# neoyinyao/Recommender

Measured on AMD Instinct MI355X. Metric: examples/sec fwd+bwd, Criteo-DLRM 26×40M×128 batch 65536, 1/2/4/8 GPU, higher is better.
Workload: dtype fp32; 1 GPU; dlrm_criteo_26x40000000x128; global_batch=65536, per_gpu_batch=65536, rows=40000000, dim=128, slots=26, optimizer=sgd, parallelism=single, prefetch=False

## Files before the change

recommender_amd/csrc/embedding.hip:

```cpp
#include <cstdlib>

#include "common.hpp"

namespace rs {

int32_t radix_sort_pairs(uint32_t*, int32_t*, uint32_t*, int32_t*, int64_t, int64_t, void*, size_t,
                         hipStream_t);
size_t radix_sort_ws_size(int64_t);
int32_t exclusive_scan_i32(const int32_t*, int32_t*, int64_t, int32_t*, void*, size_t, hipStream_t);
size_t exclusive_scan_ws_size(int64_t);

template <int VEC>
struct RowIO;
template <>
struct RowIO<4> {
  static __device__ __forceinline__ void load(const float* p, float (&v)[4]) {
    float4 t = *reinterpret_cast<const float4*>(p);
    v[0] = t.x; v[1] = t.y; v[2] = t.z; v[3] = t.w;
  }
  static __device__ __forceinline__ void store(float* p, const float (&v)[4]) {
    *reinterpret_cast<float4*>(p) = make_float4(v[0], v[1], v[2], v[3]);
  }
};
template <int VEC>
// ... 257 lines not shown

__device__ __forceinline__ int32_t seg_id_of(const ApplyArgs& a, const uint32_t* keys, int64_t k) {
  bool head = (k == 0) || keys[k - 1] != keys[k];
  return a.seg_excl ? a.seg_excl[k] + (head ? 1 : 0) - 1 : 0;
}

#ifndef RS_APPLY_BLOCKS_PER_CU
#define RS_APPLY_BLOCKS_PER_CU (1 << 20)
#endif
constexpr int kApplyBlocksPerCU = RS_APPLY_BLOCKS_PER_CU;

template <int OPT, int VEC, int CPL>
__device__ __forceinline__ void seg_tile_one(const uint32_t* __restrict__ keys,
                                             const int32_t* __restrict__ pos, int64_t n,
                                             uint32_t n_rows, const float* __restrict__ grad,
                                             const ApplyArgs& a, int lpr_log2, int64_t t);

template <int OPT, int VEC, int CPL>
__global__ __launch_bounds__(256) void seg_tile_kernel(const uint32_t* __restrict__ keys,
                                                       const int32_t* __restrict__ pos, int64_t n,
                                                       uint32_t n_rows, const float* __restrict__ grad,
                                                       ApplyArgs a, int lpr_log2, int64_t n_tiles) {
  const int gpb = blockDim.x >> lpr_log2;
  const int64_t groups = (int64_t)gridDim.x * gpb;
  for (int64_t t = (int64_t)blockIdx.x * gpb + (threadIdx.x >> lpr_log2); t < n_tiles; t += groups)
    seg_tile_one<OPT, VEC, CPL>(keys, pos, n, n_rows, grad, a, lpr_log2, t);
}

template <int OPT, int VEC, int CPL>
__device__ __forceinline__ void seg_tile_one(const uint32_t* __restrict__ keys,
                                             const int32_t* __restrict__ pos, int64_t n,
                                             uint32_t n_rows, const float* __restrict__ grad,
                                             const ApplyArgs& a, int lpr_log2, int64_t t) {
  constexpr int T = RS_DEDUP_TILE;
  constexpr int U = 8;
  const int lpr = 1 << lpr_log2;
  const int gl = threadIdx.x & (lpr - 1);
  const int64_t k0 = t * T;
  const int64_t k1 = k0 + T < n ? k0 + T : n;
  const int dim = a.dim;

  uint32_t run_row = keys[k0];
  int64_t run_start = k0;
  bool run_starts = (k0 == 0) || keys[k0 - 1] != run_row;
  const float* grad0 = (OPT == OPT_DENSE && a.n_gseg > 0) ? a.gseg[0] : grad;
  float acc[CPL][VEC];
#pragma unroll
  for (int c = 0; c < CPL; ++c)
#pragma unroll
    for (int e = 0; e < VEC; ++e) acc[c][e] = 0.f;

  auto emit = [&](uint32_t row, bool starts, bool ends, int64_t head_k) {
    if (row >= n_rows) return;
    if (starts && ends) {
      finalize_row<OPT, VEC, CPL>(a, row, gl, lpr, acc, OPT == OPT_EMIT ? seg_id_of(a, keys, head_k) : 0);
    } else {
      float* dst = a.partial + ((t * 2) + (starts ? 1 : 0)) * (int64_t)dim;
#pragma unroll
      for (int c = 0; c < CPL; ++c) {
        int col = (gl + c * lpr) * VEC;
        if (col < dim) RowIO<VEC>::store(dst + col, acc[c]);
      }
    }
  };

  for (int64_t kb = k0; kb < k1; kb += U) {
    float r[U][CPL][VEC];
    float sc[U];
    uint32_t kk[U];
    uint32_t kr[U];
    int32_t pr[U];
#pragma unroll
    for (int u = 0; u < U; ++u) {
      const int64_t k = kb + u < k1 ? kb + u : k0;
      kr[u] = keys[k];
      pr[u] = pos[k];
    }
    const float* rsp = a.row_scale ? a.row_scale : grad0;
    float sr[U];
#pragma unroll
    for (int u = 0; u < U; ++u) {
      const bool valid = kb + u < k1;
      kk[u] = valid ? kr[u] : 0xFFFFFFFFu;
      const int64_t p = valid ? pr[u] : 0;
      const bool live = valid && kk[u] < n_rows;
      sr[u] = rsp[a.row_scale && live ? p / a.scale_group : 0];
#pragma unroll
      for (int c = 0; c < CPL; ++c) {
        int col = (gl + c * lpr) * VEC;
        const bool ok = live && col < dim;
        if constexpr (OPT == OPT_DENSE)
          load_stream<VEC>(ok ? dense_grad_row(a, grad, p, dim) + col : grad0, r[u][c]);
        else
          load_stream<VEC>(ok ? grad + p * dim + col : grad0, r[u][c]);
      }
    }
#pragma unroll
    for (int u = 0; u < U; ++u) sc[u] = a.row_scale ? sr[u] : 1.f;
#pragma unroll
    for (int u = 0; u < U; ++u) {
      int64_t k = kb + u;
      if (k < k1) {
        if (kk[u] != run_row) {
          emit(run_row, run_starts, true, run_start);
#pragma unroll
          for (int c = 0; c < CPL; ++c)
#pragma unroll
            for (int e = 0; e < VEC; ++e) acc[c][e] = 0.f;
          run_row = kk[u];
          run_starts = true;
          run_start = k;
        }
        if (a.row_scale) {
#pragma unroll
          for (int c = 0; c < CPL; ++c)
#pragma unroll
            for (int e = 0; e < VEC; ++e) acc[c][e] += __fmul_rn(sc[u], r[u][c][e]);
        } else {
#pragma unroll
          for (int c = 0; c < CPL; ++c)
#pragma unroll
            for (int e = 0; e < VEC; ++e) acc[c][e] += r[u][c][e];
        }
      }
    }
  }
  bool ends = (k1 >= n) || keys[k1] != run_row;
  emit(run_row, run_starts, ends, run_start);
  if (gl == 0) {
    uint8_t f = 0;
    if (!ends && run_starts && run_row < n_rows) f |= 1;
    const uint32_t fk = keys[k0];
    if ((t % 32) == 0 && k0 > 0 && fk < n_rows && keys[k0 - 1] == fk) f |= 2;
    a.tile_flags[t] = f;
  }
}

struct Tile32Edges {
  uint32_t last_row;
  bool last_open;
  bool first_cont;
  uint32_t first_key;
};

template <int OPT, int Q = 0>
__device__ __forceinline__ Tile32Edges tile32_walk(const uint32_t* __restrict__ keys,
                                                   const int32_t* __restrict__ pos, int64_t n,
                                                   uint32_t n_rows, const float* __restrict__ grad,
                                                   const ApplyArgs& a, int64_t t, float* pbase) {
  constexpr int T = 32, VEC = 4, CPL = 1, U = 8;
  constexpr bool kQueue = Q > 0 && OPT == OPT_SGD;
  constexpr int QN = Q > 0 ? Q : 1;
  const int gl = threadIdx.x & 31;
  const int64_t k0 = t * T;
  const int64_t k1 = k0 + T < n ? k0 + T : n;
  const int ne = (int)(k1 - k0);
  const int dim = a.dim;
  const int col = gl * VEC;
  const bool mine = gl < ne;
  const uint32_t klo = a.key_lo, kspan = n_rows - a.key_lo;
  auto key_ok = [&](uint32_t k) { return k - klo < kspan; };
  const int64_t ki = k0 + (mine ? gl : 0);
  const uint32_t kraw = keys[ki];
  const int32_t praw = pos[ki];
  const uint32_t kbraw = keys[k0 > 0 ? k0 - 1 : 0];
  const uint32_t karaw = keys[k1 < n ? k1 : n - 1];
  const uint32_t kv = mine ? kraw : 0xFFFFFFFFu;
  const int32_t pv = mine ? praw : 0;
  const bool lv = mine && key_ok(kv);
  const uint32_t key_before = k0 > 0 ? kbraw : 0xFFFFFFFFu;
  const uint32_t key_after = k1 < n ? karaw : 0xFFFFFFFEu;
  float sv = 1.f;
  if (a.row_scale) sv = a.row_scale[(lv ? pv : 0) / a.scale_group];
  auto key_of = [&](int u) { return (uint32_t)__shfl((int)kv, u, 32); };
  auto load_batch = [&](int b0, float (&r)[U][VEC]) {
#pragma unroll
    for (int u = 0; u < U; ++u) {
      const int e = b0 + u;
      const int32_t p = __shfl(pv, e, 32);
      const bool live = e < ne && key_ok(key_of(e));
      load_stream<VEC>(grad + (live ? (int64_t)p * dim : 0) + col, r[u]);
    }
  };
  uint32_t run_row = key_of(0);
  int run_start = 0;
  bool run_starts = run_row != key_before;
  float acc[CPL][VEC];
#pragma unroll
  for (int c = 0; c < VEC; ++c) acc[0][c] = 0.f;
  uint32_t qrow[QN];
  float qacc[QN][VEC];
  int qn = 0;
  auto flush = [&]() {
    if constexpr (kQueue) {
      float tr[QN][VEC];
#pragma unroll
      for (int i = 0; i < QN; ++i) {
        const uint32_t rr = i < qn ? qrow[i] : (qn > 0 ? qrow[0] : 0u);
        RowIO<VEC>::load(a.table + (int64_t)rr * dim + col, tr[i]);
      }
#pragma unroll
      for (int i = 0; i < QN; ++i) {
        if (i < qn) {
#pragma unroll
          for (int c = 0; c < VEC; ++c) tr[i][c] = tr[i][c] - a.p.lr * qacc[i][c];
          RowIO<VEC>::store(a.table + (int64_t)qrow[i] * dim + col, tr[i]);
        }
      }
      qn = 0;
    }
  };
  auto emit = [&](uint32_t row, bool starts, bool ends, int head_e) {
    if (!key_ok(row)) return;
    if (starts && ends) {
      if constexpr (kQueue) {
        if (qn == QN) flush();
#pragma unroll
        for (int i = 0; i < QN; ++i) {
          if (i == qn) {
            qrow[i] = row;
#pragma unroll
            for (int c = 0; c < VEC; ++c) qacc[i][c] = acc[0][c];
          }
        }
        ++qn;
      } else {
        finalize_row<OPT, VEC, CPL>(a, row, gl, 32, acc, OPT == OPT_EMIT ? seg_id_of(a, keys, k0 + head_e) : 0);
      }
    } else {
      RowIO<VEC>::store(pbase + (starts ? 1 : 0) * dim + col, acc[0]);
    }
  };
  float rA[U][VEC], rB[U][VEC];
  load_batch(0, rA);
  auto consume = [&](int b0, float (&r)[U][VEC]) {
#pragma unroll
    for (int u = 0; u < U; ++u) {
      const int e = b0 + u;
      if (e < ne) {
        const uint32_t ku = key_of(e);
        if (ku != run_row) {
          emit(run_row, run_starts, true, run_start);
#pragma unroll
          for (int c = 0; c < VEC; ++c) acc[0][c] = 0.f;
          run_row = ku;
          run_starts = true;
          run_start = e;
        }
        if (a.row_scale) {
          const float sc = __shfl(sv, e, 32);
#pragma unroll
          for (int c = 0; c < VEC; ++c) acc[0][c] += __fmul_rn(sc, r[u][c]);
        } else {
#pragma unroll
          for (int c = 0; c < VEC; ++c) acc[0][c] += r[u][c];
        }
      }
    }
  };
#ifndef RS_T32_SINGLE
  load_batch(U, rB);
  consume(0, rA);
  if (ne > 2 * U) load_batch(2 * U, rA);
  consume(U, rB);
  if (ne > 3 * U) load_batch(3 * U, rB);
  if (ne > 2 * U) consume(2 * U, rA);
  if (ne > 3 * U) consume(3 * U, rB);
#else
  consume(0, rA);
  for (int b0 = U; b0 < ne; b0 += U) {
    load_batch(b0, rA);
    consume(b0, rA);
  }
#endif
  const bool ends = key_after != run_row;
  emit(run_row, run_starts, ends, run_start);
  flush();
  Tile32Edges ed;
  ed.last_row = run_row;
  ed.last_open = !ends && run_starts && key_ok(run_row);
  ed.first_key = key_of(0);
  ed.first_cont = k0 > 0 && key_ok(ed.first_key) && key_before == ed.first_key;
  return ed;
}

template <int OPT>
__global__ __launch_bounds__(256) void seg_tile32_kernel(const uint32_t* __restrict__ keys,
                                                         const int32_t* __restrict__ pos, int64_t n,
                                                         uint32_t n_rows,
                                                         const float* __restrict__ grad,
                                                         ApplyArgs a, int64_t n_tiles) {
  const int64_t t = (int64_t)blockIdx.x * 8 + (threadIdx.x >> 5);
  if (t >= n_tiles) return;
  const Tile32Edges e = tile32_walk<OPT>(keys, pos, n, n_rows, grad, a, t,
                                         a.partial + t * 2 * (int64_t)a.dim);
  if ((threadIdx.x & 31) == 0) {
    uint8_t f = 0;
    if (e.last_open) f |= 1;
    if ((t % 32) == 0 && e.first_cont) f |= 2;
    a.tile_flags[t] = f;
  }
}

template <int OPT, int Q = 0>
__global__ __launch_bounds__(1024) void seg_group32_kernel(const uint32_t* __restrict__ keys,
                                                           const int32_t* __restrict__ pos,
                                                           int64_t n, uint32_t n_rows,
                                                           const float* __restrict__ grad,
                                                           ApplyArgs a, int64_t n_tiles) {
  constexpr int G = 32, D = 128, T = 32;
  __shared__ __attribute__((aligned(16))) float ps[G][2][D];
  __shared__ uint32_t fkey[G];
  __shared__ int skip;
  const int gi = threadIdx.x >> 5, gl = threadIdx.x & 31;
  const int64_t t = (int64_t)blockIdx.x * G + gi;
  const bool live = t < n_tiles;
  if (a.ranged) {
    if (threadIdx.x == 0) {
      const int64_t f = (int64_t)blockIdx.x * G * T;
      const int64_t l = (f + (int64_t)G * T < n ? f + (int64_t)G * T : n) - 1;
      skip = f < n && (keys[l] < a.key_lo || keys[f] >= n_rows);
    }
    __syncthreads();
    if (skip) {
      if (gl == 0 && live) a.tile_flags[t] = 0;
      return;
    }
  }
  Tile32Edges e{};
  if (live) e = tile32_walk<OPT, Q>(keys, pos, n, n_rows, grad, a, t, &ps[gi][0][0]);
  if (gl == 0) fkey[gi] = live ? e.first_key : 0xFFFFFFFFu;
  __syncthreads();
  if (!live) return;
  const int col = gl * 4;
  uint8_t gflag = 0;
  if (e.last_open) {
    const uint32_t row = e.last_row;
    float acc[1][4];
    {
      const float4 h = *reinterpret_cast<const float4*>(&ps[gi][1][col]);
      acc[0][0] = h.x; acc[0][1] = h.y; acc[0][2] = h.z; acc[0][3] = h.w;
    }
    int u = gi + 1;
    for (; u < G && fkey[u] == row; ++u) {
      const float4 c = *reinterpret_cast<const float4*>(&ps[u][0][col]);
      acc[0][0] += c.x; acc[0][1] += c.y; acc[0][2] += c.z; acc[0][3] += c.w;
    }
    const int64_t tn = ((int64_t)blockIdx.x + 1) * G;
    const bool crosses = u == G && tn < n_tiles && keys[tn * T] == row;
    if (crosses) {
      RowIO<4>::store(a.chunk + (t * 2 + 1) * (int64_t)D + col, acc[0]);
      gflag = 1;
    } else {
      finalize_row<OPT, 4, 1>(a, row, gl, 32, acc,
                              OPT == OPT_EMIT ? seg_id_of(a, keys, t * T + T - 1) : 0);
    }
  }
  if (gi == 0 && e.first_cont) {
    const uint32_t fk = e.first_key;
    float acc[4];
    {
      const float4 h = *reinterpret_cast<const float4*>(&ps[0][0][col]);
      acc[0] = h.x; acc[1] = h.y; acc[2] = h.z; acc[3] = h.w;
    }
    for (int u = 1; u < G && fkey[u] == fk; ++u) {
      const float4 c = *reinterpret_cast<const float4*>(&ps[u][0][col]);
      acc[0] += c.x; acc[1] += c.y; acc[2] += c.z; acc[3] += c.w;
    }
    RowIO<4>::store(a.chunk + (t * 2) * (int64_t)D + col, acc);
  }
  if (gl == 0) a.tile_flags[t] = gflag;
}

constexpr int kFixChunk = 32;

template <int VEC, int CPL>
__device__ __forceinline__ void load_or_zero(const float* p, int dim, int gl, int lpr,
                                             float (&acc)[CPL][VEC]) {
#pragma unroll
  for (int c = 0; c < CPL; ++c) {
    int col = (gl + c * lpr) * VEC;
    if (col < dim) {
      RowIO<VEC>::load(p + col, acc[c]);
    } else {
#pragma unroll
      for (int e = 0; e < VEC; ++e) acc[c][e] = 0.f;
    }
  }
}

template <int VEC, int CPL>
__device__ __forceinline__ void store_row(float* p, int dim, int gl, int lpr,
                                          const float (&acc)[CPL][VEC]) {
#pragma unroll
  for (int c = 0; c < CPL; ++c) {
    int col = (gl + c * lpr) * VEC;
    if (col < dim) RowIO<VEC>::store(p + col, acc[c]);
  }
}

template <int VEC, int CPL>
__device__ __forceinline__ void fold_group(const uint32_t* keys, int64_t n, uint32_t key,
                                           const float* part, int64_t t1, int64_t t_end, int dim,
                                           int gl, int lpr, float (&acc)[CPL][VEC]) {
  constexpr int T = RS_DEDUP_TILE;
  constexpr int U = 8;
  for (int64_t t = t1; t < t_end; t += U) {
    bool in[U];
    float r[U][CPL][VEC];
#pragma unroll
    for (int u = 0; u < U; ++u) {
      const int64_t tt = t + u;
      in[u] = tt < t_end && tt * T < n && keys[tt * T] == key;
    }
    bool more = true;
#pragma unroll
    for (int u = 0; u < U; ++u) {
      more = more && in[u];
      in[u] = more;
    }
#pragma unroll
    for (int u = 0; u < U; ++u) {
      if (in[u]) {
        load_or_zero<VEC, CPL>(part + ((t + u) * 2) * (int64_t)dim, dim, gl, lpr, r[u]);
      }
    }
#pragma unroll
    for (int u = 0; u < U; ++u)
      if (in[u])
#pragma unroll
        for (int c = 0; c < CPL; ++c)
#pragma unroll
          for (int e = 0; e < VEC; ++e) acc[c][e] += r[u][c][e];
    if (!more) return;
  }
}

template <int VEC, int CPL>
__global__ __launch_bounds__(256) void seg_chunk_kernel(const uint32_t* __restrict__ keys, int64_t n,
                                                        uint32_t n_rows, ApplyArgs a, int lpr_log2,
                                                        int64_t n_tiles, float* __restrict__ chunk) {
  constexpr int T = RS_DEDUP_TILE;
  const int lpr = 1 << lpr_log2;
  const int gl = threadIdx.x & (lpr - 1);
  const int64_t t = (int64_t)blockIdx.x * (blockDim.x >> lpr_log2) + (threadIdx.x >> lpr_log2);
  if (t >= n_tiles) return;
  const uint8_t flags = a.tile_flags[t];
  if (flags == 0) return;
  const int dim = a.dim;
  const int64_t k0 = t * T;
  const int64_t klast = (k0 + T < n ? k0 + T : n) - 1;
  const int64_t group_end = (t / kFixChunk + 1) * kFixChunk;
  float acc[CPL][VEC];
  if (flags & 1) {
    const uint32_t lk = keys[klast];
    load_or_zero<VEC, CPL>(a.partial + (t * 2 + 1) * (int64_t)dim, dim, gl, lpr, acc);
    fold_group<VEC, CPL>(keys, n, lk, a.partial, t + 1, group_end, dim, gl, lpr, acc);
    store_row<VEC, CPL>(chunk + (t * 2 + 1) * (int64_t)dim, dim, gl, lpr, acc);
  }
  if (flags & 2) {
    const uint32_t fk = keys[k0];
    load_or_zero<VEC, CPL>(a.partial + (t * 2) * (int64_t)dim, dim, gl, lpr, acc);
    fold_group<VEC, CPL>(keys, n, fk, a.partial, t + 1, group_end, dim, gl, lpr, acc);
    store_row<VEC, CPL>(chunk + (t * 2) * (int64_t)dim, dim, gl, lpr, acc);
  }
}

template <int OPT, int VEC, int CPL>
__device__ __forceinline__ void fixup_one(const uint32_t* __restrict__ keys, const ApplyArgs& a,
                                          int lpr_log2, int64_t n_tiles,
                                          const float* __restrict__ chunk, int64_t t);

template <int OPT, int VEC, int CPL>
__global__ __launch_bounds__(256) void seg_fixup_kernel(const uint32_t* __restrict__ keys, int64_t n,
                                                        uint32_t n_rows, ApplyArgs a, int lpr_log2,
                                                        int64_t n_tiles,
                                                        const float* __restrict__ chunk) {
  const int64_t t = (int64_t)blockIdx.x * (blockDim.x >> lpr_log2) + (threadIdx.x >> lpr_log2);
  if (t >= n_tiles - 1) return;
  if (!(a.tile_flags[t] & 1)) return;
  fixup_one<OPT, VEC, CPL>(keys, a, lpr_log2, n_tiles, chunk, t);
}

template <int OPT, int VEC, int CPL>
__global__ __launch_bounds__(256) void seg_fixup_wave_kernel(const uint32_t* __restrict__ keys,
                                                             ApplyArgs a, int lpr_log2,
                                                             int64_t n_tiles,
                                                             const float* __restrict__ chunk) {
  constexpr int T = RS_DEDUP_TILE;
  constexpr int U = 16;
  const int64_t t = (int64_t)blockIdx.x * 4 + (threadIdx.x >> 6);
  if (t >= n_tiles - 1) return;
  if (!(a.tile_flags[t] & 1)) return;
  const int lane = threadIdx.x & 63;
  const int lpr = 1 << lpr_log2;
  const int nlg = 64 >> lpr_log2;
  const int lg = lane >> lpr_log2, gl = lane & (lpr - 1);
  const int64_t klast = t * T + T - 1;
  const uint32_t row = keys[klast];
  const int dim = a.dim;
  float acc[CPL][VEC];
  load_or_zero<VEC, CPL>(chunk + (t * 2 + 1) * (int64_t)dim, dim, gl, lpr, acc);
  const int span = nlg * U < 64 ? nlg * U : 64;
  for (int64_t g = t / kFixChunk + 1;; g += span) {
    uint32_t k[U];
    float r[U][CPL][VEC];
    uint32_t mine = 0;
#pragma unroll
    for (int u = 0; u < U; ++u) {
      const int64_t gg = g + (int64_t)lg * U + u;
      const int64_t tt = gg * kFixChunk;
      const bool in = lg * U + u < span && tt < n_tiles;
      k[u] = in ? keys[tt * T] : ~row;
      if (in)
        load_or_zero<VEC, CPL>(chunk + (tt * 2) * (int64_t)dim, dim, gl, lpr, r[u]);
      else
#pragma unroll
        for (int c = 0; c < CPL; ++c)
#pragma unroll
          for (int e = 0; e < VEC; ++e) r[u][c][e] = 0.f;
      mine |= (k[u] == row ? 1u : 0u) << u;
    }
    uint64_t w = 0;
    for (int src = 0; src < nlg && src * U < span; ++src)
      w |= (uint64_t)(uint32_t)__shfl((int)mine, src * lpr) << (src * U);
    const int nrun = ~w == 0ull ? 64 : (int)__builtin_ctzll(~w);
    for (int src = 0; src < nlg && src * U < nrun; ++src) {
#pragma unroll
      for (int u = 0; u < U; ++u) {
        float v[CPL][VEC];
#pragma unroll
        for (int c = 0; c < CPL; ++c)
#pragma unroll
          for (int e = 0; e < VEC; ++e) v[c][e] = __shfl(r[u][c][e], src * lpr + gl);
        if (src * U + u < nrun)
#pragma unroll
          for (int c = 0; c < CPL; ++c)
#pragma unroll
            for (int e = 0; e < VEC; ++e) acc[c][e] += v[c][e];
      }
    }
    if (nrun < span) break;
  }
  if (lg == 0) finalize_row<OPT, VEC, CPL>(a, row, gl, lpr, acc, OPT == OPT_EMIT ? seg_id_of(a, keys, klast) : 0);
}

template <int OPT>
__global__ __launch_bounds__(256) void seg_fixup_sweep_kernel(const uint32_t* __restrict__ keys,
                                                              ApplyArgs a, int64_t n_tiles,
                                                              const float* __restrict__ chunk) {
  const int gl = threadIdx.x & 31;
  const int64_t groups = (int64_t)gridDim.x * 8;
  for (int64_t t0 = ((int64_t)blockIdx.x * 8 + (threadIdx.x >> 5)) * 32; t0 < n_tiles - 1;
       t0 += groups * 32) {
    const int64_t tl = t0 + gl;
    const bool head = tl < n_tiles - 1 && (a.tile_flags[tl] & 1);
    uint32_t bits = (uint32_t)(__ballot(head) >> (threadIdx.x & 32));
    while (bits) {
      const int u = __builtin_ctz(bits);
      bits &= bits - 1;
      fixup_one<OPT, 4, 1>(keys, a, 5, n_tiles, chunk, t0 + u);
    }
  }
}

template <int OPT, int VEC, int CPL>
__device__ __forceinline__ void fixup_one(const uint32_t* __restrict__ keys, const ApplyArgs& a,
                                          int lpr_log2, int64_t n_tiles,
                                          const float* __restrict__ chunk, int64_t t) {
  constexpr int T = RS_DEDUP_TILE;
  constexpr int U = 16;
  const int lpr = 1 << lpr_log2;
  const int gl = threadIdx.x & (lpr - 1);
  const int64_t klast = t * T + T - 1;
  const uint32_t row = keys[klast];
  const int dim = a.dim;
  float acc[CPL][VEC];
  load_or_zero<VEC, CPL>(chunk + (t * 2 + 1) * (int64_t)dim, dim, gl, lpr, acc);
  for (int64_t g = t / kFixChunk + 1;; g += U) {
    bool in[U];
    float r[U][CPL][VEC];
    bool more = true;
    uint32_t k[U];
#pragma unroll
    for (int u = 0; u < U; ++u) {
      const int64_t tt = (g + u) * kFixChunk;
      k[u] = tt < n_tiles ? keys[tt * T] : ~row;
      if (tt < n_tiles)
        load_or_zero<VEC, CPL>(chunk + ((g + u) * kFixChunk * 2) * (int64_t)dim, dim, gl, lpr, r[u]);
    }
#pragma unroll
    for (int u = 0; u < U; ++u) {
      in[u] = more && k[u] == row;
      more = in[u];
    }
#pragma unroll
    for (int u = 0; u < U; ++u)
      if (in[u])
#pragma unroll
        for (int c = 0; c < CPL; ++c)
#pragma unroll
          for (int e = 0; e < VEC; ++e) acc[c][e] += r[u][c][e];
    if (!more) break;
  }
  finalize_row<OPT, VEC, CPL>(a, row, gl, lpr, acc, OPT == OPT_EMIT ? seg_id_of(a, keys, klast) : 0);
}

__global__ void head_flags_kernel(const uint32_t* __restrict__ keys, int64_t n, uint32_t n_rows,
                                  int32_t* __restrict__ flags) {
  int64_t i = blockIdx.x * (int64_t)blockDim.x + threadIdx.x;
  int64_t stride = (int64_t)gridDim.x * blockDim.x;
  for (; i < n; i += stride) {
    uint32_t k = keys[i];
    flags[i] = (k < n_rows && (i == 0 || keys[i - 1] != k)) ? 1 : 0;
  }
}

__device__ __forceinline__ void keras_decay(float& w, float& m, float& v, float lr, float b1,
                                            float b2, float eps) {
  const float m1 = m * b1;
  const float v1 = v * b2;
  const float upd = (lr * m1) / (sqrtf(v1) + eps);
  m = m1;
  v = v1;
  w = w - upd;
}

template <int VEC>
__device__ __forceinline__ bool keras_state_zero(const float (&mm)[VEC], const float (&vv)[VEC]) {
  bool z = true;
#pragma unroll
  for (int e = 0; e < VEC; ++e) z &= (__float_as_uint(mm[e]) == 0u) & (vv[e] == 0.0f);
  return z;
}

template <int VEC>
__global__ __launch_bounds__(256) void keras_dense_sweep_kernel(float* __restrict__ w,
                                                                float* __restrict__ m,
                                                                float* __restrict__ v, int64_t n_rows,
                                                                int dim, rs_adam_params p,
                                                                const uint32_t* __restrict__ bitmap) {
  const int64_t chunks_per_row = dim / VEC;
  const int64_t total = n_rows * chunks_per_row;
  int64_t i = blockIdx.x * (int64_t)blockDim.x + threadIdx.x;
  const int64_t stride = (int64_t)gridDim.x * blockDim.x;
  for (; i < total; i += stride) {
    int64_t row = i / chunks_per_row;
    if ((bitmap[row >> 5] >> (row & 31)) & 1u) continue;
    int64_t off = i * VEC;
    float ww[VEC], mm[VEC], vv[VEC];
    RowIO<VEC>::load(m + off, mm);
    RowIO<VEC>::load(v + off, vv);
    if (keras_state_zero<VEC>(mm, vv)) continue;
    RowIO<VEC>::load(w + off, ww);
#pragma unroll
    for (int e = 0; e < VEC; ++e) keras_decay(ww[e], mm[e], vv[e], p.lr, p.beta1, p.beta2, p.epsilon);
    RowIO<VEC>::store(w + off, ww);
    RowIO<VEC>::store(m + off, mm);
    RowIO<VEC>::store(v + off, vv);
  }
}

template <int VEC>
__device__ __forceinline__ void keras_replay_row(float* w, float* m, float* v, int64_t r, int dim,
                                                 int gl, int lpr, int32_t from, int32_t to,
                                                 const float* lr_hist, float b1, float b2,
                                                 float eps) {
  for (int col = gl * VEC; col < dim; col += lpr * VEC) {
    const int64_t off = r * dim + col;
    float ww[VEC], mm[VEC], vv[VEC];
    RowIO<VEC>::load(m + off, mm);
    RowIO<VEC>::load(v + off, vv);
    if (keras_state_zero<VEC>(mm, vv)) continue;
    RowIO<VEC>::load(w + off, ww);
    for (int32_t st = from; st <= to; ++st) {
      const float lr = lr_hist[st];
#pragma unroll
      for (int e = 0; e < VEC; ++e) keras_decay(ww[e], mm[e], vv[e], lr, b1, b2, eps);
    }
    RowIO<VEC>::store(w + off, ww);
    RowIO<VEC>::store(m + off, mm);
    RowIO<VEC>::store(v + off, vv);
  }
}

template <int VEC>
__global__ __launch_bounds__(256) void keras_catchup_kernel(
    float* __restrict__ w, float* __restrict__ m, float* __restrict__ v, int32_t* __restrict__ last,
    uint32_t n_rows, int dim, const uint32_t* __restrict__ rows, int64_t n,
    const float* __restrict__ lr_hist, int32_t step, float b1, float b2, float eps, int lpr_log2) {
  const int lpr = 1 << lpr_log2;
  const int gl = threadIdx.x & (lpr - 1);
  const int64_t stride = ((int64_t)gridDim.x * blockDim.x) >> lpr_log2;
  for (int64_t i = ((int64_t)blockIdx.x * blockDim.x + threadIdx.x) >> lpr_log2; i < n; i += stride) {
    const uint32_t r = rows[i];
    if (r >= n_rows || (i > 0 && rows[i - 1] == r)) continue;
    const int32_t l0 = last[r];
    if (l0 + 1 <= step - 1)
      keras_replay_row<VEC>(w, m, v, r, dim, gl, lpr, l0 + 1, step - 1, lr_hist, b1, b2, eps);
    if (gl == 0) last[r] = step - 1;
  }
}

__global__ __launch_bounds__(256) void keras_mark_kernel(int32_t* __restrict__ last, uint32_t n_rows,
                                                          const uint32_t* __restrict__ rows,
                                                          int64_t n, int32_t step) {
  for (int64_t i = (int64_t)blockIdx.x * blockDim.x + threadIdx.x; i < n;
       i += (int64_t)gridDim.x * blockDim.x) {
    const uint32_t r = rows[i];
    if (r < n_rows && (i == 0 || rows[i - 1] != r)) last[r] = step;
  }
}

template <int VEC>
__global__ __launch_bounds__(256) void keras_materialize_kernel(
    float* __restrict__ w, float* __restrict__ m, float* __restrict__ v, int32_t* __restrict__ last,
    int64_t n_rows, int dim, const float* __restrict__ lr_hist, int32_t step, float b1, float b2,
    float eps, int lpr_log2) {
  const int lpr = 1 << lpr_log2;
  const int gl = threadIdx.x & (lpr - 1);
  const int64_t stride = ((int64_t)gridDim.x * blockDim.x) >> lpr_log2;
  for (int64_t r = ((int64_t)blockIdx.x * blockDim.x + threadIdx.x) >> lpr_log2; r < n_rows; r += stride) {
    const int32_t l0 = last[r];
    if (l0 + 1 <= step)
      keras_replay_row<VEC>(w, m, v, r, dim, gl, lpr, l0 + 1, step, lr_hist, b1, b2, eps);
    if (gl == 0) last[r] = step;
  }
}

template <template <int, int> class K>
struct Noop {};

#define RS_DISPATCH_VEC_CPL(geom, CALL)                                   \
  do {                                                                    \
    switch ((geom).vec * 100 + (geom).cpl) {                              \
      case 401: { constexpr int VEC = 4, CPL = 1; CALL; } break;          \
      case 402: { constexpr int VEC = 4, CPL = 2; CALL; } break;          \
      case 404: { constexpr int VEC = 4, CPL = 4; CALL; } break;          \
      case 408: { constexpr int VEC = 4, CPL = 8; CALL; } break;          \
      case 201: { constexpr int VEC = 2, CPL = 1; CALL; } break;          \
      case 202: { constexpr int VEC = 2, CPL = 2; CALL; } break;          \
      case 204: { constexpr int VEC = 2, CPL = 4; CALL; } break;          \
      case 101: { constexpr int VEC = 1, CPL = 1; CALL; } break;          \
      case 102: { constexpr int VEC = 1, CPL = 2; CALL; } break;          \
      case 104: { constexpr int VEC = 1, CPL = 4; CALL; } break;          \
      default:                                                            \
        set_error("row geometry vec=%d cpl=%d unsupported (dim too large)", (geom).vec, (geom).cpl); \
        return RS_E_UNSUPPORTED;                                          \
    }                                                                     \
  } while (0)

__global__ __launch_bounds__(256) void keras_bitmap_mark_kernel(const uint32_t* __restrict__ keys,
                                                               int64_t n, uint32_t n_rows,
                                                               uint32_t* __restrict__ bitmap) {
  for (int64_t k = (int64_t)blockIdx.x * 256 + threadIdx.x; k < n; k += (int64_t)gridDim.x * 256) {
    const uint32_t row = keys[k];
    if (row < n_rows && (k == 0 || keys[k - 1] != row)) atomicOr(bitmap + (row >> 5), 1u << (row & 31));
  }
}

#ifndef RS_SGD_QUEUE
#define RS_SGD_QUEUE 2
#endif

static int32_t launch_segments(int opt, const uint32_t* keys, const int32_t* pos, int64_t n,
                               int64_t n_rows, const float* grad, const ApplyArgs& a,
                               const RowGeom& geom, hipStream_t st) {
  const int64_t n_tiles = ceil_div(n, RS_DEDUP_TILE);
  const int gpb = 256 >> geom.lpr_log2;
  const int64_t blocks = ceil_div(n_tiles, gpb);
  if (blocks == 0) return RS_OK;
  static int cus = 0;
  if (!cus) {
    int dev = 0;
    if (hipGetDevice(&dev) != hipSuccess ||
        hipDeviceGetAttribute(&cus, hipDeviceAttributeMultiprocessorCount, dev) != hipSuccess)
      cus = 256;
  }
  const int64_t walk_blocks = std::min<int64_t>(blocks, (int64_t)cus * kApplyBlocksPerCU);
#ifndef RS_NO_T32
  const bool t32 = geom.vec == 4 && geom.cpl == 1 && geom.lpr_log2 == 5 && RS_DEDUP_TILE == 32;
#else
  const bool t32 = false;
#endif
#ifndef RS_NO_G32
  const bool g32 = t32;
#else
  const bool g32 = false;
#endif
  if (a.key_lo && !g32) {
    set_error("a key range needs the D = 128 group walk (16-byte aligned rows)");
    return RS_E_UNSUPPORTED;
  }
#define RS_SEG_LAUNCH(OPTV)                                                                     \
  RS_DISPATCH_VEC_CPL(geom, ({                                                                  \
    if (g32) {                                                                                  \
      if (OPTV == OPT_SGD)                                                                      \
        seg_group32_kernel<OPTV, RS_SGD_QUEUE><<<ceil_div(n_tiles, 32), 1024, 0, st>>>(         \
            keys, pos, n, (uint32_t)n_rows, grad, a, n_tiles);                                  \
      else                                                                                      \
        seg_group32_kernel<OPTV><<<ceil_div(n_tiles, 32), 1024, 0, st>>>(keys, pos, n,          \
                                                                     (uint32_t)n_rows, grad, a, \
                                                                     n_tiles);                  \
    } else {                                                                                    \
      if (t32)                                                                                  \
        seg_tile32_kernel<OPTV><<<ceil_div(n_tiles, 8), 256, 0, st>>>(       \
            keys, pos, n, (uint32_t)n_rows, grad, a, n_tiles);                                  \
      else                                                                                      \
        seg_tile_kernel<OPTV, VEC, CPL><<<walk_blocks, 256, 0, st>>>(                           \
            keys, pos, n, (uint32_t)n_rows, grad, a, geom.lpr_log2, n_tiles);                   \
      seg_chunk_kernel<VEC, CPL><<<blocks, 256, 0, st>>>(keys, n, (uint32_t)n_rows, a,          \
                                                         geom.lpr_log2, n_tiles, a.chunk);      \
    }                                                                                           \
    if (g32)                                                                                    \
      seg_fixup_sweep_kernel<OPTV><<<(unsigned)std::min<int64_t>(ceil_div(n_tiles, 256), 1024),  \
                                     256, 0, st>>>(keys, a, n_tiles, a.chunk);                  \
    else                                                                                        \
      seg_fixup_wave_kernel<OPTV, VEC, CPL><<<(unsigned)ceil_div(n_tiles, 4), 256, 0, st>>>(    \
          keys, a, geom.lpr_log2, n_tiles, a.chunk);                                            \
  }))
  switch (opt) {
    case OPT_SGD: RS_SEG_LAUNCH(OPT_SGD); break;
    case OPT_LAZY: RS_SEG_LAUNCH(OPT_LAZY); break;
    case OPT_ADAGRAD: RS_SEG_LAUNCH(OPT_ADAGRAD); break;
    case OPT_ROWWISE: RS_SEG_LAUNCH(OPT_ROWWISE); break;
    case OPT_KERAS:
      RS_SEG_LAUNCH(OPT_KERAS);
      keras_bitmap_mark_kernel<<<(unsigned)std::min<int64_t>(ceil_div(n, 256), 2048), 256, 0, st>>>(
          keys, n, (uint32_t)n_rows, a.bitmap);
      break;
    case OPT_EMIT: RS_SEG_LAUNCH(OPT_EMIT); break;
    case OPT_DENSE: RS_SEG_LAUNCH(OPT_DENSE); break;
    default: set_error("unknown optimizer %d", opt); return RS_E_INVALID;
  }
#undef RS_SEG_LAUNCH
  RS_CHECK_LAUNCH();
  return RS_OK;
}

}

using namespace rs;

extern "C" int32_t rs_embedding_fwd_strided(const float* table, int64_t n_rows, int32_t dim,
                                            const void* ids, int32_t id_dtype, int64_t n_ids,
                                            const int64_t* slot_offsets, int32_t n_slots, float* out,
                                            int64_t out_ld, int32_t* err_flag, void* stream);

extern "C" int32_t rs_embedding_fwd(const float* table, int64_t n_rows, int32_t dim, const void* ids,
                                    int32_t id_dtype, int64_t n_ids, const int64_t* slot_offsets,
                                    int32_t n_slots, float* out, int32_t* err_flag, void* stream) {
  return rs_embedding_fwd_strided(table, n_rows, dim, ids, id_dtype, n_ids, slot_offsets, n_slots,
                                  out, dim, err_flag, stream);
}

extern "C" int32_t rs_embedding_fwd_strided(const float* table, int64_t n_rows, int32_t dim,
                                            const void* ids, int32_t id_dtype, int64_t n_ids,
                                            const int64_t* slot_offsets, int32_t n_slots, float* out,
                                            int64_t out_ld, int32_t* err_flag, void* stream) {
  RS_CHECK_ARG(dim > 0, "dim must be > 0");
  RS_CHECK_ARG(out_ld >= dim, "out_ld must be >= dim");
  RS_CHECK_ARG(n_ids >= 0, "n_ids must be >= 0");
  RS_CHECK_ARG(n_slots >= 1, "n_slots must be >= 1");
  RS_CHECK_ARG(id_dtype == RS_ID_I32 || id_dtype == RS_ID_I64, "bad id dtype");
  RS_CHECK_ARG(n_ids == 0 || (table && ids && out), "null pointer");
  if (n_ids == 0) return RS_OK;
  hipStream_t st = as_stream(stream);
  if (out_ld == dim && dim % 4 != 0 && dim % 2 == 0 && dim <= 64 &&
      ((reinterpret_cast<uintptr_t>(table) | reinterpret_cast<uintptr_t>(out)) & 7) == 0) {
    const int64_t pairs = n_ids * dim / 2;
    const int blocks = (int)std::min<int64_t>(ceil_div(pairs, 256), 256 * 32);
    gather_flat2_kernel<<<blocks, 256, 0, st>>>(table, n_rows, dim, ids, id_dtype, n_ids,
                                                slot_offsets, n_slots, out, err_flag);
    RS_CHECK_LAUNCH();
    return RS_OK;
  }
  const void* ptrs[3] = {table, out, reinterpret_cast<const void*>((uintptr_t)(out_ld * 4))};
  RowGeom geom = row_geom(dim, ptrs, 3);
  const int gpb = 256 >> geom.lpr_log2;
  int64_t blocks = std::min<int64_t>(ceil_div(n_ids, gpb * 4), 256 * 16);
  RS_DISPATCH_VEC_CPL(geom, ({
    gather_kernel<VEC, CPL><<<blocks, 256, 0, st>>>(table, n_rows, dim, ids, id_dtype, n_ids,
                                                    slot_offsets, n_slots, out, err_flag,
                                                    geom.lpr_log2, out_ld);
  }));
  RS_CHECK_LAUNCH();
  return RS_OK;
}

static size_t partial_bytes(int64_t n_ids, int32_t dim) {
  return 2 * align_up((size_t)ceil_div(n_ids, RS_DEDUP_TILE) * 2 * dim * sizeof(float), 256) +
         align_up((size_t)ceil_div(n_ids, RS_DEDUP_TILE), 256);
}
static uint8_t* flags_of(float* partial, int64_t n_ids, int32_t dim) {
  return reinterpret_cast<uint8_t*>(partial) +
         2 * align_up((size_t)ceil_div(n_ids, RS_DEDUP_TILE) * 2 * dim * sizeof(float), 256);
}
static float* chunk_of(float* partial, int64_t n_ids, int32_t dim) {
  return partial + align_up((size_t)ceil_div(n_ids, RS_DEDUP_TILE) * 2 * dim * sizeof(float), 256) / 4;
}

extern "C" size_t rs_dedup_workspace_size(int64_t n_ids, int32_t dim) {
  return align_up(partial_bytes(n_ids, dim), 256) + align_up((size_t)n_ids * 4, 256) +
         exclusive_scan_ws_size(n_ids) + 256;
}

extern "C" int32_t rs_embedding_dedup_grad_scaled(const uint32_t* sorted_rows,
                                                  const int32_t* sorted_pos, int64_t n_ids,
                                                  const float* grad_out, const float* row_scale,
                                                  int32_t scale_group, int32_t dim, int64_t n_rows,
                                                  uint32_t* uniq_rows, float* uniq_grad,
                                                  void* workspace, size_t ws_bytes, void* stream);

extern "C" int32_t rs_embedding_dedup_grad(const uint32_t* sorted_rows, const int32_t* sorted_pos,
                                           int64_t n_ids, const float* grad_out, int32_t dim,
                                           int64_t n_rows, uint32_t* uniq_rows, float* uniq_grad,
                                           void* workspace, size_t ws_bytes, void* stream) {
  return rs_embedding_dedup_grad_scaled(sorted_rows, sorted_pos, n_ids, grad_out, nullptr, 1, dim,
                                        n_rows, uniq_rows, uniq_grad, workspace, ws_bytes, stream);
}

extern "C" int32_t rs_embedding_dedup_grad_mapped(const uint32_t* sorted_rows,
                                                  const int32_t* sorted_pos, int64_t n_ids,
                                                  const float* grad_out, const float* row_scale,
                                                  int32_t scale_group, int32_t dim, int64_t n_rows,
                                                  const int32_t* seg_map, uint32_t* uniq_rows,
                                                  float* uniq_grad, void* workspace,
                                                  size_t ws_bytes, void* stream);

extern "C" int32_t rs_embedding_dedup_grad_scaled(const uint32_t* sorted_rows,
                                                  const int32_t* sorted_pos, int64_t n_ids,
                                                  const float* grad_out, const float* row_scale,
                                                  int32_t scale_group, int32_t dim, int64_t n_rows,
                                                  uint32_t* uniq_rows, float* uniq_grad,
                                                  void* workspace, size_t ws_bytes, void* stream) {
  return rs_embedding_dedup_grad_mapped(sorted_rows, sorted_pos, n_ids, grad_out, row_scale,
                                        scale_group, dim, n_rows, nullptr, uniq_rows, uniq_grad,
                                        workspace, ws_bytes, stream);
}

extern "C" int32_t rs_embedding_dedup_grad_mapped_range(
    const uint32_t* sorted_rows, const int32_t* sorted_pos, int64_t n_ids, const float* grad_out,
    const float* row_scale, int32_t scale_group, int32_t dim, int64_t n_rows, uint32_t key_lo,
    uint32_t key_hi, int32_t seg_ready, const int32_t* seg_excl, const int32_t* seg_map,
    uint32_t* uniq_rows,
    float* uniq_grad, void* workspace, size_t ws_bytes, void* stream);

extern "C" int32_t rs_embedding_dedup_grad_mapped(const uint32_t* sorted_rows,
                                                  const int32_t* sorted_pos, int64_t n_ids,
                                                  const float* grad_out, const float* row_scale,
                                                  int32_t scale_group, int32_t dim, int64_t n_rows,
                                                  const int32_t* seg_map, uint32_t* uniq_rows,
                                                  float* uniq_grad, void* workspace,
                                                  size_t ws_bytes, void* stream) {
  return rs_embedding_dedup_grad_mapped_range(sorted_rows, sorted_pos, n_ids, grad_out, row_scale,
                                              scale_group, dim, n_rows, 0u, (uint32_t)n_rows, 0,
                                              nullptr, seg_map, uniq_rows, uniq_grad, workspace,
                                              ws_bytes, stream);
}

extern "C" int32_t rs_embedding_dedup_grad_mapped_range(
    const uint32_t* sorted_rows, const int32_t* sorted_pos, int64_t n_ids, const float* grad_out,
    const float* row_scale, int32_t scale_group, int32_t dim, int64_t n_rows, uint32_t key_lo,
    uint32_t key_hi, int32_t seg_ready, const int32_t* seg_excl, const int32_t* seg_map,
    uint32_t* uniq_rows,
    float* uniq_grad, void* workspace, size_t ws_bytes, void* stream) {
  RS_CHECK_ARG(dim > 0 && n_ids >= 0 && n_rows > 0, "bad sizes");
  RS_CHECK_ARG(key_lo < key_hi && (int64_t)key_hi <= n_rows, "key range outside [0, n_rows)");
  RS_CHECK_ARG(!row_scale || scale_group >= 1, "scale_group must be >= 1");
  if (n_ids == 0) return RS_OK;
  RS_CHECK_ARG(sorted_rows && sorted_pos && grad_out && uniq_rows && uniq_grad, "null pointer");
  if (ws_bytes < rs_dedup_workspace_size(n_ids, dim)) {
    set_error("dedup workspace too small");
    return RS_E_WORKSPACE;
  }
  hipStream_t st = as_stream(stream);
  Carver c(workspace, ws_bytes);
  float* partial = c.take<float>(partial_bytes(n_ids, dim) / 4);
  int32_t* seg = c.take<int32_t>(n_ids);
  void* scan_ws = c.take<char>(exclusive_scan_ws_size(n_ids));
  int blocks = (int)std::min<int64_t>(ceil_div(n_ids, 256), 4096);
  if (seg_excl) {
    seg = const_cast<int32_t*>(seg_excl);
  } else if (!seg_ready) {
    head_flags_kernel<<<blocks, 256, 0, st>>>(sorted_rows, n_ids, (uint32_t)n_rows, seg);
    RS_CHECK_LAUNCH();
    int32_t s = exclusive_scan_i32(seg, seg, n_ids, nullptr, scan_ws, exclusive_scan_ws_size(n_ids), st);
    if (s) return s;
  }
  ApplyArgs a{};
  a.dim = dim;
  a.partial = partial;
  a.chunk = chunk_of(partial, n_ids, dim);
  a.tile_flags = flags_of(partial, n_ids, dim);
  a.uniq_grad = uniq_grad;
  a.uniq_rows = uniq_rows;
  a.seg_excl = seg;
  a.row_scale = row_scale;
  a.scale_group = scale_group;
  a.seg_map = seg_map;
  a.key_lo = key_lo;
  a.ranged = key_lo != 0 || (int64_t)key_hi < n_rows;
  const void* ptrs[2] = {grad_out, uniq_grad};
  RowGeom geom = row_geom(dim, ptrs, 2);
  return launch_segments(OPT_EMIT, sorted_rows, sorted_pos, n_ids, key_hi, grad_out, a, geom, st);
}

extern "C" int32_t rs_embedding_grad_dense(const uint32_t* sorted_rows, const int32_t* sorted_pos,
                                           int64_t n_ids, const float* grad_out, int32_t dim,
                                           int64_t n_rows, float* dense, void* workspace,
                                           size_t ws_bytes, void* stream) {
  RS_CHECK_ARG(dim > 0 && n_ids >= 0 && n_rows > 0, "bad sizes");
  RS_CHECK_ARG(dense, "null pointer");
  hipStream_t st = as_stream(stream);
  RS_CHECK_HIP(hipMemsetAsync(dense, 0, (size_t)n_rows * dim * sizeof(float), st));
  if (n_ids == 0) return RS_OK;
  RS_CHECK_ARG(sorted_rows && sorted_pos && grad_out, "null pointer");
  if (ws_bytes < partial_bytes(n_ids, dim)) {
    set_error("dense-gradient workspace too small");
    return RS_E_WORKSPACE;
  }
  ApplyArgs a{};
  a.table = dense;
  a.dim = dim;
  a.partial = static_cast<float*>(workspace);
  a.chunk = chunk_of(a.partial, n_ids, dim);
  a.tile_flags = flags_of(a.partial, n_ids, dim);
  const void* ptrs[2] = {grad_out, dense};
  RowGeom geom = row_geom(dim, ptrs, 2);
  return launch_segments(OPT_DENSE, sorted_rows, sorted_pos, n_ids, n_rows, grad_out, a, geom, st);
}

extern "C" int32_t rs_embedding_grad_dense_segs(const uint32_t* sorted_rows,
                                                const int32_t* sorted_pos, int64_t n_ids,
                                                int32_t n_segs, const float* const* seg_ptrs,
                                                const int64_t* seg_n, const int64_t* seg_ld,
                                                int32_t dim, int64_t n_rows, float* dense,
                                                void* workspace, size_t ws_bytes, void* stream) {
  RS_CHECK_ARG(dim > 0 && n_ids >= 0 && n_rows > 0, "bad sizes");
  RS_CHECK_ARG(n_segs >= 1 && n_segs <= 4, "1..4 gradient segments");
  RS_CHECK_ARG(dense && seg_ptrs && seg_n && seg_ld, "null pointer");
  ApplyArgs a{};
  int64_t total = 0;
  const void* ptrs[9];
  int np = 0;
  for (int i = 0; i < n_segs; ++i) {
    RS_CHECK_ARG(seg_n[i] >= 0 && seg_ld[i] >= dim, "segment rows >= 0, row stride >= dim");
    RS_CHECK_ARG(seg_n[i] == 0 || seg_ptrs[i], "null segment pointer");
    a.gseg[i] = seg_ptrs[i];
    a.gstart[i] = total;
    a.gld[i] = seg_ld[i];
    total += seg_n[i];
    ptrs[np++] = seg_ptrs[i];
    ptrs[np++] = reinterpret_cast<const void*>((uintptr_t)seg_ld[i] * 4);
  }
  RS_CHECK_ARG(total == n_ids, "segment rows must sum to n_ids");
  a.n_gseg = n_segs;
  hipStream_t st = as_stream(stream);
  RS_CHECK_HIP(hipMemsetAsync(dense, 0, (size_t)n_rows * dim * sizeof(float), st));
  if (n_ids == 0) return RS_OK;
  RS_CHECK_ARG(sorted_rows && sorted_pos, "null pointer");
  if (ws_bytes < partial_bytes(n_ids, dim)) {
    set_error("dense-gradient workspace too small");
    return RS_E_WORKSPACE;
  }
  a.table = dense;
  a.dim = dim;
  a.partial = static_cast<float*>(workspace);
  a.chunk = chunk_of(a.partial, n_ids, dim);
  a.tile_flags = flags_of(a.partial, n_ids, dim);
  ptrs[np++] = dense;
  RowGeom geom = row_geom(dim, ptrs, np);
  if (geom.vec == 4 && geom.cpl == 1 && geom.lpr_log2 == 5) geom.vec = 2, geom.lpr_log2 = 6;
  return launch_segments(OPT_DENSE, sorted_rows, sorted_pos, n_ids, n_rows, a.gseg[0], a, geom, st);
}

extern "C" size_t rs_apply_workspace_size(int64_t n_ids, int32_t dim) {
  return align_up(partial_bytes(n_ids, dim), 256) + 256;
}

extern "C" int32_t rs_embedding_apply_scaled(int32_t opt, float* table, float* m, float* v,
                                             int64_t n_rows, int32_t dim,
                                             const uint32_t* sorted_rows, const int32_t* sorted_pos,
                                             int64_t n_ids, const float* grad_out,
                                             const float* row_scale, int32_t scale_group,
                                             const rs_adam_params* params,
                                             uint32_t* touched_bitmap, void* workspace,
                                             size_t ws_bytes, void* stream);

extern "C" int32_t rs_embedding_apply(int32_t opt, float* table, float* m, float* v, int64_t n_rows,
                                      int32_t dim, const uint32_t* sorted_rows,
                                      const int32_t* sorted_pos, int64_t n_ids,
                                      const float* grad_out, const rs_adam_params* params,
                                      uint32_t* touched_bitmap, void* workspace, size_t ws_bytes,
                                      void* stream) {
  return rs_embedding_apply_scaled(opt, table, m, v, n_rows, dim, sorted_rows, sorted_pos, n_ids,
                                   grad_out, nullptr, 1, params, touched_bitmap, workspace,
                                   ws_bytes, stream);
}

extern "C" int32_t rs_embedding_apply_scaled(int32_t opt, float* table, float* m, float* v,
                                             int64_t n_rows, int32_t dim,
                                             const uint32_t* sorted_rows, const int32_t* sorted_pos,
                                             int64_t n_ids, const float* grad_out,
                                             const float* row_scale, int32_t scale_group,
                                             const rs_adam_params* params,
// ... 304 lines not shown
```

Baseline: 103.5 million examples/sec.

## Run group32 apply kernel with fewer threads, each half-wave walking multiple tiles

The group32 segment-apply kernel is templated on the number of half-waves per block. For SGD and the other non-lazy optimizers it now launches 512 threads per block instead of 1024, with each half-wave walking two tiles in sequence. Per-tile edge state (last row, flags) moves into shared memory so the cross-tile merge can loop over several tiles per half-wave. A min-blocks-per-CU launch bound of 4 is added. The aim is more resident blocks and better latency hiding per CU, at the cost of serialising tile walks inside each half-wave and possible register pressure from the launch bound.

```diff
diff --git a/recommender_amd/csrc/embedding.hip b/recommender_amd/csrc/embedding.hip
--- a/recommender_amd/csrc/embedding.hip
+++ b/recommender_amd/csrc/embedding.hip
@@ -583,19 +583,21 @@
   }
 }
 
-template <int OPT, int Q = 0>
-__global__ __launch_bounds__(1024) void seg_group32_kernel(const uint32_t* __restrict__ keys,
-                                                           const int32_t* __restrict__ pos,
-                                                           int64_t n, uint32_t n_rows,
-                                                           const float* __restrict__ grad,
-                                                           ApplyArgs a, int64_t n_tiles) {
+template <int OPT, int Q = 0, int HW = 32>
+__global__ __launch_bounds__(HW * 32, 4) void seg_group32_kernel(const uint32_t* __restrict__ keys,
+                                                                 const int32_t* __restrict__ pos,
+                                                                 int64_t n, uint32_t n_rows,
+                                                                 const float* __restrict__ grad,
+                                                                 ApplyArgs a, int64_t n_tiles) {
+  static_assert(HW == 32 || HW == 16 || HW == 8, "half-waves per block: 32, 16 or 8");
   constexpr int G = 32, D = 128, T = 32;
   __shared__ __attribute__((aligned(16))) float ps[G][2][D];
   __shared__ uint32_t fkey[G];
+  __shared__ uint32_t lrow[G];
+  __shared__ uint8_t edge[G];
   __shared__ int skip;
   const int gi = threadIdx.x >> 5, gl = threadIdx.x & 31;
-  const int64_t t = (int64_t)blockIdx.x * G + gi;
-  const bool live = t < n_tiles;
+  const int64_t t0 = (int64_t)blockIdx.x * G;
   if (a.ranged) {
     if (threadIdx.x == 0) {
       const int64_t f = (int64_t)blockIdx.x * G * T;
@@ -604,53 +606,77 @@
     }
     __syncthreads();
     if (skip) {
-      if (gl == 0 && live) a.tile_flags[t] = 0;
+      if (gl == 0)
+        for (int j = gi; j < G && t0 + j < n_tiles; j += HW) a.tile_flags[t0 + j] = 0;
       return;
     }
   }
-  Tile32Edges e{};
-  if (live) e = tile32_walk<OPT, Q>(keys, pos, n, n_rows, grad, a, t, &ps[gi][0][0]);
-  if (gl == 0) fkey[gi] = live ? e.first_key : 0xFFFFFFFFu;
+  auto walk_tile = [&](const int j) {
+    const int64_t t = t0 + j;
+    if (t < n_tiles) {
+      const Tile32Edges e = tile32_walk<OPT, Q>(keys, pos, n, n_rows, grad, a, t, &ps[j][0][0]);
+      if (gl == 0) {
+        fkey[j] = e.first_key;
+        lrow[j] = e.last_row;
+        edge[j] = (uint8_t)((e.last_open ? 1 : 0) | (e.first_cont ? 2 : 0));
+      }
+    } else if (gl == 0) {
+      fkey[j] = 0xFFFFFFFFu;
+      edge[j] = 0;
+    }
+  };
+  if constexpr (HW == G) {
+    walk_tile(gi);
+  } else {
+#pragma unroll
+    for (int r = 0; r < G / HW; ++r) walk_tile(r * HW + gi);
+  }
   __syncthreads();
-  if (!live) return;
   const int col = gl * 4;
-  uint8_t gflag = 0;
-  if (e.last_open) {
-    const uint32_t row = e.last_row;
-    float acc[1][4];
-    {
-      const float4 h = *reinterpret_cast<const float4*>(&ps[gi][1][col]);
-      acc[0][0] = h.x; acc[0][1] = h.y; acc[0][2] = h.z; acc[0][3] = h.w;
-    }
-    int u = gi + 1;
-    for (; u < G && fkey[u] == row; ++u) {
-      const float4 c = *reinterpret_cast<const float4*>(&ps[u][0][col]);
-      acc[0][0] += c.x; acc[0][1] += c.y; acc[0][2] += c.z; acc[0][3] += c.w;
-    }
-    const int64_t tn = ((int64_t)blockIdx.x + 1) * G;
-    const bool crosses = u == G && tn < n_tiles && keys[tn * T] == row;
-    if (crosses) {
-      RowIO<4>::store(a.chunk + (t * 2 + 1) * (int64_t)D + col, acc[0]);
-      gflag = 1;
-    } else {
-      finalize_row<OPT, 4, 1>(a, row, gl, 32, acc,
-                              OPT == OPT_EMIT ? seg_id_of(a, keys, t * T + T - 1) : 0);
-    }
-  }
-  if (gi == 0 && e.first_cont) {
-    const uint32_t fk = e.first_key;
-    float acc[4];
-    {
-      const float4 h = *reinterpret_cast<const float4*>(&ps[0][0][col]);
-      acc[0] = h.x; acc[1] = h.y; acc[2] = h.z; acc[3] = h.w;
-    }
-    for (int u = 1; u < G && fkey[u] == fk; ++u) {
-      const float4 c = *reinterpret_cast<const float4*>(&ps[u][0][col]);
-      acc[0] += c.x; acc[1] += c.y; acc[2] += c.z; acc[3] += c.w;
-    }
-    RowIO<4>::store(a.chunk + (t * 2) * (int64_t)D + col, acc);
-  }
-  if (gl == 0) a.tile_flags[t] = gflag;
+#pragma unroll 1
+  for (int r = 0; r < G / HW; ++r) {
+    const int j = r * HW + gi;
+    const int64_t t = t0 + j;
+    if (t >= n_tiles) return;
+    const uint8_t ej = edge[j];
+    uint8_t gflag = 0;
+    if (ej & 1) {
+      const uint32_t row = lrow[j];
+      float acc[1][4];
+      {
+        const float4 h = *reinterpret_cast<const float4*>(&ps[j][1][col]);
+        acc[0][0] = h.x; acc[0][1] = h.y; acc[0][2] = h.z; acc[0][3] = h.w;
+      }
+      int u = j + 1;
+      for (; u < G && fkey[u] == row; ++u) {
+        const float4 c = *reinterpret_cast<const float4*>(&ps[u][0][col]);
+        acc[0][0] += c.x; acc[0][1] += c.y; acc[0][2] += c.z; acc[0][3] += c.w;
+      }
+      const int64_t tn = t0 + G;
+      const bool crosses = u == G && tn < n_tiles && keys[tn * T] == row;
+      if (crosses) {
+        RowIO<4>::store(a.chunk + (t * 2 + 1) * (int64_t)D + col, acc[0]);
+        gflag = 1;
+      } else {
+        finalize_row<OPT, 4, 1>(a, row, gl, 32, acc,
+                                OPT == OPT_EMIT ? seg_id_of(a, keys, t * T + T - 1) : 0);
+      }
+    }
+    if (j == 0 && (ej & 2)) {
+      const uint32_t fk = fkey[0];
+      float acc[4];
+      {
+        const float4 h = *reinterpret_cast<const float4*>(&ps[0][0][col]);
+        acc[0] = h.x; acc[1] = h.y; acc[2] = h.z; acc[3] = h.w;
+      }
+      for (int u = 1; u < G && fkey[u] == fk; ++u) {
+        const float4 c = *reinterpret_cast<const float4*>(&ps[u][0][col]);
+        acc[0] += c.x; acc[1] += c.y; acc[2] += c.z; acc[3] += c.w;
+      }
+      RowIO<4>::store(a.chunk + (t * 2) * (int64_t)D + col, acc);
+    }
+    if (gl == 0) a.tile_flags[t] = gflag;
+  }
 }
 
 constexpr int kFixChunk = 32;
@@ -1043,6 +1069,12 @@
 #ifndef RS_SGD_QUEUE
 #define RS_SGD_QUEUE 2
 #endif
+#ifndef RS_APPLY_HW
+#define RS_APPLY_HW 16
+#endif
+constexpr int apply_hw(int opt) {
+  return opt == OPT_LAZY || opt == OPT_KERAS || opt == OPT_ADAGRAD ? 32 : RS_APPLY_HW;
+}
 
 static int32_t launch_segments(int opt, const uint32_t* keys, const int32_t* pos, int64_t n,
                                int64_t n_rows, const float* grad, const ApplyArgs& a,
@@ -1077,12 +1109,13 @@
   RS_DISPATCH_VEC_CPL(geom, ({                                                                  \
     if (g32) {                                                                                  \
       if (OPTV == OPT_SGD)                                                                      \
-        seg_group32_kernel<OPTV, RS_SGD_QUEUE><<<ceil_div(n_tiles, 32), 1024, 0, st>>>(         \
-            keys, pos, n, (uint32_t)n_rows, grad, a, n_tiles);                                  \
+        seg_group32_kernel<OPTV, RS_SGD_QUEUE, apply_hw(OPTV)>                                  \
+            <<<ceil_div(n_tiles, 32), apply_hw(OPTV) * 32, 0, st>>>(                            \
+                keys, pos, n, (uint32_t)n_rows, grad, a, n_tiles);                              \
       else                                                                                      \
-        seg_group32_kernel<OPTV><<<ceil_div(n_tiles, 32), 1024, 0, st>>>(keys, pos, n,          \
-                                                                     (uint32_t)n_rows, grad, a, \
-                                                                     n_tiles);                  \
+        seg_group32_kernel<OPTV, 0, apply_hw(OPTV)>                                             \
+            <<<ceil_div(n_tiles, 32), apply_hw(OPTV) * 32, 0, st>>>(                            \
+                keys, pos, n, (uint32_t)n_rows, grad, a, n_tiles);                              \
     } else {                                                                                    \
       if (t32)                                                                                  \
         seg_tile32_kernel<OPTV><<<ceil_div(n_tiles, 8), 256, 0, st>>>(       \
```

Result: faster. 105.7 million examples/sec (median of 6 runs) (+2.1%).
